# DaehwanKimLab/tophat

Hardware: AMD Instinct MI355X
Metric: paired reads/sec through segment_juncs+long_spanning_reads; junctions.bed diff=0 (higher is better)
Workload: dtype u64

## Files before the change

### tophat_amd/csrc/thj_core.h

```cpp
#pragma once
#include <stdint.h>

#if defined(__HIPCC__)
#define THJ_HD __host__ __device__ __forceinline__
#else
#define THJ_HD inline
#endif

#if defined(THJ_EXP) && defined(__HIPCC__)
static __device__ int thj_exp_flags;
#define THJ_EXPF(b) (thj_exp_flags & (b))
#else
#define THJ_EXPF(b) 0
#endif

namespace thj {

typedef unsigned long long u64;

THJ_HD int popc(u64 x) { return __builtin_popcountll(x); }
THJ_HD int popc32(uint32_t x) { return __builtin_popcount(x); }
THJ_HD int ctz(u64 x) { return __builtin_ctzll(x); }
THJ_HD int clz(u64 x) { return __builtin_clzll(x); }
THJ_HD u64 lowmask(int n) { return n >= 64 ? ~0ull : ((1ull << n) - 1ull); }
// ... 652 lines not shown
    bool run = nseg > 0;
    if (last == 0) run = run && (present & 1u) && !hit_end(h[0]);
    bool check_partner = true;
    if (last != 0 && (present & 1u) && h[0].ref_id == hl.ref_id && hit_anti(h[0]) == hit_anti(hl)) {
        const int dist = hit_anti(h[0]) ? h[0].left - hl.right : hl.left - h[0].right;
        if (dist >= p.min_segment_intron && dist < p.max_segment_intron) check_partner = false;
    }
    res.rescue = run && check_partner && n_mate > 0;
    bool en = run && !res.rescue;
    if (p.bowtie2 && present != 0 && 1 > p.max_seg_multihits) en = false;
#pragma unroll
    for (int s = 0; s + 1 < NS; ++s) {
        const bool has = en && s != last && ((present >> s) & 1u);
        const Hit bh = h[s];
        const bool banti = hit_anti(bh);
        const Hit rh = h[s + 1];
        const bool c1 = ((present >> (s + 1)) & 1u) && banti == hit_anti(rh) && bh.ref_id == rh.ref_id;
        const bool abut = banti ? rh.right == bh.left : bh.right == rh.left;
        const int d1 = banti ? bh.left - rh.right : rh.left - bh.right;
        const bool found = c1 && abut;
        const bool drs = c1 && !abut && d1 >= p.min_segment_intron && d1 < p.max_segment_intron;
        bool rrs = false;
        Hit d = rh;
        if (s + 2 < NS) {
            const Hit rrh = h[s + 2];
            const bool c2 = ((present >> (s + 2)) & 1u) && banti == hit_anti(rrh) && bh.ref_id == rrh.ref_id;
            const int d2 = banti ? bh.left - rrh.right : rrh.left - bh.right;
            rrs = !found && c2 && d2 >= p.min_segment_intron + L && d2 < p.max_segment_intron + L;
            if (rrs) d = rrh;
        }
        const int start = (s + 1) * L - 8;
        int slen = rrs ? L + 16 : 16;
        if (slen > rl - start) slen = rl - start;
        int32_t wl, wr;
        if (!banti) { wl = bh.right - 8; if (wl < 0) wl = 0; wr = d.left + 8; }
        else { wl = d.right - 8; wr = bh.left + 8; }
        const bool ok = has && !found && (drs || rrs) && start >= 0 && slen >= 0;
        emit.task(ok, task_window_word(banti, start, slen), bh.ref_id, (uint32_t)wl, (uint32_t)wr);
        res.n_windows += ok ? 1 : 0;
    }
    return res;
}

enum { SLOT_UNSCANNED = -3 };
template <int MAXM, class Emit>
THJ_HD int flat_rescue(const Params& p, bool has0, const Hit& bh, int size, int rl, const Hit (&mh)[MAXM], int n_mate,
                       const int32_t (&sc)[2 * MAXM], Emit& emit, int& n_windows) {
    const int L = p.segment_length;
    int cl = L - p.segment_mismatches - 3;
    if (cl > 15) cl = 15;
    const bool banti = hit_anti(bh);
    bool alive = has0;
    int pairs = 0, n_pseudo = 0;
    int32_t pl[2 * MAXM];
    bool pv[2 * MAXM];
#pragma unroll
    for (int m = 0; m < MAXM; ++m) {
        const bool compat = alive && m < n_mate && bh.ref_id == mh[m].ref_id && banti != hit_anti(mh[m]);
        const int32_t f = compat ? sc[2 * m] : SLOT_NONE, rv = compat ? sc[2 * m + 1] : SLOT_NONE;
        if (compat && f == SLOT_BREAK) alive = false;
        pairs += (compat && f != SLOT_BREAK && f != SLOT_UNSCANNED) ? 1 : 0;
        pv[2 * m] = compat && alive && f >= 0; pl[2 * m] = f;
        pv[2 * m + 1] = compat && alive && rv >= 0; pl[2 * m + 1] = rv;
        n_pseudo += (pv[2 * m] ? 1 : 0) + (pv[2 * m + 1] ? 1 : 0);
    }
    bool en = has0 && (size == 2 || size == 3);
    if (p.bowtie2 && (1 > p.max_seg_multihits || n_pseudo > p.max_seg_multihits)) en = false;
    const bool far = size == 3;
    const int lo = p.min_segment_intron + (far ? L : 0), hi = p.max_segment_intron + (far ? L : 0);
    bool found = false, inr[2 * MAXM];
    int n = 0;
#pragma unroll
    for (int k = 0; k < 2 * MAXM; ++k) {
        const bool panti = (k & 1) != 0;
        const bool c = pv[k] && banti == panti;
        const int32_t pleft = pl[k], pright = pl[k] + cl;
        const bool abut = banti ? pright == bh.left : bh.right == pleft;
        if (c && abut && !far) found = true;
        const int dist = banti ? bh.left - pright : pleft - bh.right;
        inr[k] = c && dist >= lo && dist < hi;
        n += inr[k] ? 1 : 0;
    }
    const int start = L - 8;
    int slen = far ? L + 16 : 16;
    if (slen > rl - start) slen = rl - start;
    const bool ok_all = en && !found && n > 0 && start >= 0 && slen >= 0;
#pragma unroll
    for (int k = 0; k < 2 * MAXM; ++k) {
        const int32_t pleft = pl[k], pright = pl[k] + cl;
        int32_t wl, wr;
        if (!banti) { wl = bh.right - 8; if (wl < 0) wl = 0; wr = pleft + 8; }
        else { wl = pright - 8; wr = bh.left + 8; }
        const bool ok = ok_all && inr[k];
        emit.task(ok, task_window_word(banti, start, slen), bh.ref_id, (uint32_t)wl, (uint32_t)wr);
        n_windows += ok ? 1 : 0;
    }
    return pairs;
}

template <class Sink>
THJ_HD void gaps_enumerate(const Params& p, const ReadView& v, Sink& sink, int first = 0, int stride = 1) {
    const int L = p.segment_length;
    if (p.bowtie2)
        for (int s = 0; s < v.size; ++s) {
            int n = (!v.rescue || s == 0) ? rv_count_raw(v, s) : rv_count(v, s);
            if (n > p.max_seg_multihits) return;
        }
    for (int s = 0; s < v.size; ++s) {
        rv_foreach_strided(v, s, first, stride, [&](const Hit& bh) {
            bool found = (s == v.size - 1);
            int n_drs = 0, n_rrs = 0;
            const bool banti = hit_anti(bh);
            if (s < v.size - 1) {
                rv_foreach(v, s + 1, [&](const Hit& rh) {
                    if (banti != hit_anti(rh) || bh.ref_id != rh.ref_id) return true;
                    if ((banti && rh.right == bh.left) || (!banti && bh.right == rh.left)) { found = true; return false; }
                    int dist = banti ? bh.left - rh.right : rh.left - bh.right;
                    if (dist >= p.min_segment_intron && dist < p.max_segment_intron) ++n_drs;
                    return true;
                });
            }
            if (!found && s < v.size - 2) {
                rv_foreach(v, s + 2, [&](const Hit& rrh) {
                    if (banti != hit_anti(rrh) || bh.ref_id != rrh.ref_id) return true;
                    int dist = banti ? bh.left - rrh.right : rrh.left - bh.right;
                    if (dist >= p.min_segment_intron + L && dist < p.max_segment_intron + L) ++n_rrs;
                    return true;
                });
            }
            if (!found && (n_drs > 0 || n_rrs > 0)) {
                const bool use_rrs = n_rrs > 0;
                const int lo = p.min_segment_intron + (use_rrs ? L : 0);
                const int hi = p.max_segment_intron + (use_rrs ? L : 0);
                const int start = (s + 1) * L - 8;
                int slen = use_rrs ? L + 16 : 16;
                if (slen > v.rl - start) slen = v.rl - start;
                if (start >= 0 && slen >= 0) {
                    rv_foreach(v, use_rrs ? s + 2 : s + 1, [&](const Hit& d) {
                        if (banti != hit_anti(d) || bh.ref_id != d.ref_id) return true;
                        int dist = banti ? bh.left - d.right : d.left - bh.right;
                        if (dist < lo || dist >= hi) return true;
                        int32_t wl, wr;
                        if (!banti) { wl = bh.right - 8; if (wl < 0) wl = 0; wr = d.left + 8; }
                        else { wl = d.right - 8; wr = bh.left + 8; }
                        sink.window(bh.ref_id, wl, wr, banti, start, slen);
                        return true;
                    });
                }
            }
        });
    }
}

template <class X>
THJ_HD Hit wave_bcast_hit(X& x, const Hit& h, int src) {
    Hit o;
    o.ref_id = x.bcast(h.ref_id, src); o.left = (int32_t)x.bcast((uint32_t)h.left, src);
    o.right = (int32_t)x.bcast((uint32_t)h.right, src); o.meta = x.bcast(h.meta, src);
    return o;
}
THJ_HD Hit wave_lane_hit(const ReadView& v, int s, int lane) {
    Hit h{0, 0, 0, 0};
    if (lane < rv_count_raw(v, s)) h = v.hits[v.so[s] + (uint32_t)lane];
    return h;
}
THJ_HD bool wave_read_fits(const ReadView& v) {
    for (int s = 0; s < v.nseg; ++s) if (rv_count_raw(v, s) > 64) return false;
    return true;
}
template <class X, class Sink>
THJ_HD bool wave_read_enumerate(X& x, const Params& p, ReadView& v, Sink& sink, bool& wants_rescue) {
    const int lane = x.lane;
    const int L = p.segment_length;
    wants_rescue = false;
    v.rescue = false;
    v.check_len = p.segment_length - p.segment_mismatches - 3;
    if (v.check_len > 15) v.check_len = 15;
    if (v.nseg == 0) return false;
    int last = v.nseg - 1;
    while (last > 0 && rv_count_raw(v, last) == 0) --last;
    v.size = last + 1;
    if (last == 0) {
        if (rv_count_raw(v, 0) == 0) return false;
        const Hit h0 = v.hits[v.so[0]];
        if (hit_end(h0)) return false;
    }
    {
        bool found = false;
        if (last != 0) {
            const Hit lh = wave_lane_hit(v, 0, lane);
            const bool have = lane < rv_count_raw(v, 0);
            const Hit D = wave_lane_hit(v, last, lane);
            const int nD = rv_count_raw(v, last);
            for (int j = 0; j < nD; ++j) {
                const Hit rh = wave_bcast_hit(x, D, j);
                if (have && lh.ref_id == rh.ref_id && hit_anti(lh) == hit_anti(rh)) {
                    const int dist = hit_anti(lh) ? lh.left - rh.right : rh.left - lh.right;
                    if (dist >= p.min_segment_intron && dist < p.max_segment_intron) found = true;
                }
            }
        }
        wants_rescue = x.ballot(found) == 0ull && v.n_mate > 0;
    }
    if (wants_rescue) return true;
    if (THJ_EXPF(1 << 27)) return true;
    if (v.nseg >= 2 && !THJ_EXPF(1 << 17))
        for (int i = 0; i + 2 < v.nseg; ++i) {
            const uint32_t lb = v.so[i], le = v.so[i + 1], re = v.so[i + 2];
            if (lb == le || le == re) break;
            const int start = i * L;
            if (start > v.rl) break;
            const int plen = v.rl - start < 2 * L ? v.rl - start : 2 * L;
            const Hit lh = wave_lane_hit(v, i, lane);
            const bool have = (uint32_t)lane < le - lb;
            const Hit C = wave_lane_hit(v, i + 1, lane);
            const int nC = (int)(re - le);
            for (int ri = 0; ri < nC; ++ri) {
                const Hit rh = wave_bcast_hit(x, C, ri);
                if (!have || lh.ref_id != rh.ref_id) continue;
                const bool anti = hit_anti(lh);
                if (anti != hit_anti(rh)) continue;
                const int apparent = anti ? lh.right - rh.left : rh.right - lh.left;
                const int disc = apparent - plen;
                const bool is_del = disc > 0 && disc <= p.max_deletion_length;
                const bool is_ins = disc < 0 && disc >= -p.max_insertion_length;
                if (is_del || is_ins)
                    sink.indel(i, anti ? le + (uint32_t)ri : lb + (uint32_t)lane, anti ? lb + (uint32_t)lane : le + (uint32_t)ri, lane, ri, anti, plen, is_del);
            }
        }
    if (THJ_EXPF(1 << 25)) return true;
    if (p.bowtie2)
        for (int s = 0; s < v.size; ++s) if (rv_count_raw(v, s) > p.max_seg_multihits) return true;
    for (int s = 0; s + 1 < v.size; ++s) {
        const Hit bh = wave_lane_hit(v, s, lane);
        const bool have = lane < rv_count_raw(v, s);
        const bool banti = hit_anti(bh);
        const Hit B = wave_lane_hit(v, s + 1, lane);
        const int nB = rv_count_raw(v, s + 1);
        bool found = false;
        int n_drs = 0, n_rrs = 0;
        for (int c = 0; c < nB; ++c) {
            const Hit rh = wave_bcast_hit(x, B, c);
            if (!have || banti != hit_anti(rh) || bh.ref_id != rh.ref_id) continue;
            if ((banti && rh.right == bh.left) || (!banti && bh.right == rh.left)) found = true;
            const int dist = banti ? bh.left - rh.right : rh.left - bh.right;
            if (dist >= p.min_segment_intron && dist < p.max_segment_intron) ++n_drs;
        }
        Hit C{0, 0, 0, 0};
        int nC = 0;
        if (s < v.size - 2) {
            C = wave_lane_hit(v, s + 2, lane);
            nC = rv_count_raw(v, s + 2);
            if (x.ballot(have && !found) != 0ull)
                for (int c = 0; c < nC; ++c) {
                    const Hit rrh = wave_bcast_hit(x, C, c);
                    if (!have || found || banti != hit_anti(rrh) || bh.ref_id != rrh.ref_id) continue;
                    const int dist = banti ? bh.left - rrh.right : rrh.left - bh.right;
                    if (dist >= p.min_segment_intron + L && dist < p.max_segment_intron + L) ++n_rrs;
                }
        }
        const bool emits = have && !found && (n_drs > 0 || n_rrs > 0);
        const bool use_rrs = n_rrs > 0;
        const int lo = p.min_segment_intron + (use_rrs ? L : 0), hi = p.max_segment_intron + (use_rrs ? L : 0);
        const int start = (s + 1) * L - 8;
        int slen = use_rrs ? L + 16 : 16;
        if (slen > v.rl - start) slen = v.rl - start;
        const bool go = emits && start >= 0 && slen >= 0;
        for (int pass = 0; pass < 2; ++pass) {
            const bool mine = go && (use_rrs ? pass == 1 : pass == 0);
            if (x.ballot(mine) == 0ull) continue;
            const int nT = pass == 0 ? nB : nC;
            for (int c = 0; c < nT; ++c) {
                const Hit d = wave_bcast_hit(x, pass == 0 ? B : C, c);
                if (!mine || banti != hit_anti(d) || bh.ref_id != d.ref_id) continue;
                const int dist = banti ? bh.left - d.right : d.left - bh.right;
                if (dist < lo || dist >= hi) continue;
                int32_t wl, wr;
                if (!banti) { wl = bh.right - 8; if (wl < 0) wl = 0; wr = d.left + 8; }
                else { wl = d.right - 8; wr = bh.left + 8; }
                sink.window(bh.ref_id, wl, wr, banti, start, slen);
            }
        }
    }
    return true;
}

template <class Sink>
THJ_HD void indels_enumerate(const Params& p, const ReadView& v, Sink& sink, int first = 0, int stride = 1) {
    const int L = p.segment_length;
    if (v.nseg < 2) return;
    for (int i = 0; i + 2 < v.nseg; ++i) {
        uint32_t lb = v.so[i], le = v.so[i + 1], re = v.so[i + 2];
        if (lb == le || le == re) return;
        int start = i * L;
        if (start > v.rl) return;
        int plen = v.rl - start < 2 * L ? v.rl - start : 2 * L;
        for (uint32_t li = lb + (uint32_t)first; li < le; li += (uint32_t)stride) {
            Hit lh = v.hits[li];
            for (uint32_t ri = le; ri < re; ++ri) {
                Hit rh = v.hits[ri];
                if (lh.ref_id != rh.ref_id) continue;
                bool anti = hit_anti(lh);
                if (anti != hit_anti(rh)) continue;
                int apparent = anti ? lh.right - rh.left : rh.right - lh.left;
                int disc = apparent - plen;
                bool is_del = disc > 0 && disc <= p.max_deletion_length;
                bool is_ins = disc < 0 && disc >= -p.max_insertion_length;
                if (is_del || is_ins)
                    sink.indel(i, anti ? ri : li, anti ? li : ri, (int)(li - lb), (int)(ri - le), anti, plen, is_del);
            }
        }
    }
}

template <bool WIDE = true, class Sink>
THJ_HD void indel_exec(const Genome& g, const Params& p, const ReadView& v, int i, uint32_t lidx, uint32_t ridx,
                       bool anti, int plen, bool is_del, u64 prio, Sink& sink) {
    const Hit lh = v.hits[lidx], rh = v.hits[ridx];
    if (!WIDE || plen <= 64) {
        if (plen > 64) return;
        PlanesT<u64> rd = Fetch<u64>::read(v.rp, v.W, i * p.segment_length, plen);
        if (anti) rd = Fetch<u64>::rc(rd, plen);
        if (is_del) small_deletion<u64>(g, rd, plen, lh, rh, sink);
        else small_insertion<u64>(g, rd, plen, lh, rh, prio, sink);
    } else if (WIDE) {
        PlanesT<u128> rd = Fetch<u128>::read(v.rp, v.W, i * p.segment_length, plen);
        if (anti) rd = Fetch<u128>::rc(rd, plen);
        if (is_del) small_deletion<u128>(g, rd, plen, lh, rh, sink);
        else small_insertion<u128>(g, rd, plen, lh, rh, prio, sink);
    }
}

template <bool WIDE = true, class Sink>
THJ_HD void window_exec(const Genome& g, const Params& p, const ReadView& v, uint32_t ref_id, int32_t wl, int32_t wr,
                        bool anti, int start, int slen, Sink& sink) {
    if (slen < 2) return;
    if (!WIDE || slen <= 62) {
        if (slen > 62) return;
        PlanesT<u64> sup = Fetch<u64>::read(v.rp, v.W, start, slen);
        if (anti) sup = Fetch<u64>::rc(sup, slen);
        window_scan<u64>(g, p, ref_id, wl, wr, anti, sup, slen, sink);
    } else if (WIDE) {
        PlanesT<u128> sup = Fetch<u128>::read(v.rp, v.W, start, slen);
        if (anti) sup = Fetch<u128>::rc(sup, slen);
        window_scan<u128>(g, p, ref_id, wl, wr, anti, sup, slen, sink);
    }
}

static constexpr int INS_SEQ_BITS = 18;
THJ_HD u64 ins_prio(uint32_t ordinal, int i, int li, int ri) {
    if (li > 63) li = 63;
    if (ri > 63) ri = 63;
    return ((u64)ordinal << 16) | ((u64)(i & 15) << 12) | ((u64)li << 6) | (u64)ri;
}


enum { FUS_FF = 7, FUS_FR = 8, FUS_RF = 9, FUS_RR = 10 };

THJ_HD Planes read_piece(const u64* rp, int W, int rl, bool rc, int off, int len) {
    if (!rc) return r_fetch(rp, W, off, len);
    return rc_piece(r_fetch(rp, W, rl - off - len, len), len);
}
THJ_HD Planes genomic_piece(const Genome& g, uint32_t ref, int64_t start, int rl, bool rc, int off, int len) {
    if (!rc) return g_fetch(g, ref, start + off);
    Planes p = g_fetch(g, ref, start + rl - off - len);
    return rc_piece(p, len);
}

template <int NW>
struct FusEvalT { u64 mL[NW], mR[NW]; int e1, min_err, total_ed; bool lrc, rrc; };
using FusEval = FusEvalT<4>;
template <int NW>
THJ_HD int fusion_eval(const Genome& g, const Params& p, const u64* rp, int W, int rl, bool read_rc, const Hit& lh, const Hit& rh, int dir, FusEvalT<NW>& ev) {
    const int32_t llen = g_len(g, lh.ref_id), rlen = g_len(g, rh.ref_id);
    if (llen == 0 || rlen == 0 || rl > NW * 64) return 0;
    int64_t lstart, rstart;
    const bool lrc = !(dir == FUS_FF || dir == FUS_FR), rrc = !(dir == FUS_FF || dir == FUS_RF);
    ev.lrc = lrc; ev.rrc = rrc;
    if (!lrc) { if (lh.left + rl > llen || lh.left < 0) return 0; lstart = lh.left; }
    else { if (lh.right < rl || lh.right > llen) return 0; lstart = (int64_t)lh.right - rl; }
    if (!rrc) { if (rh.right < rl || rh.right > rlen) return 0; rstart = (int64_t)rh.right - rl; }
    else { if (rh.left + rl > rlen || rh.left < 0) return 0; rstart = rh.left; }
    int tot_r = 0;
#pragma unroll
    for (int w = 0; w < NW; ++w) {
        ev.mL[w] = 0; ev.mR[w] = 0;
        int off = w * 64;
        if (off < rl) {
            int l = rl - off < 64 ? rl - off : 64;
            Planes rd = read_piece(rp, W, rl, read_rc, off, l);
            Planes a = genomic_piece(g, lh.ref_id, lstart, rl, lrc, off, l);
            Planes b = genomic_piece(g, rh.ref_id, rstart, rl, rrc, off, l);
            u64 M = lowmask(l);
            ev.mL[w] = ((a.lo ^ rd.lo) | (a.hi ^ rd.hi) | a.nm | rd.nm) & M;
            ev.mR[w] = ((b.lo ^ rd.lo) | (b.hi ^ rd.hi) | b.nm | rd.nm) & M;
            tot_r += popc(ev.mR[w]);
        }
    }
    ev.e1 = (int)(ev.mL[0] & 1ull) + tot_r - (int)(ev.mR[0] & 1ull);
    ev.total_ed = hit_ed(lh) + hit_ed(rh);
    const int A = p.fusion_anchor_length;
    int mn = rl + 1, cnt = 0, mn_ends = rl + 1, ee = ev.e1;
#pragma unroll
    for (int w = 0; w < NW; ++w) {
        const int q0 = w == 0 ? 1 : w * 64, q1 = rl < (w + 1) * 64 ? rl : (w + 1) * 64;
        u64 l = ev.mL[w] >> (q0 & 63), r = ev.mR[w] >> (q0 & 63);
        for (int q = q0; q < q1; ++q) {
            if (ee < mn) { mn = ee; cnt = 1; } else if (ee == mn) ++cnt;
            if ((q < A || rl - q < A) && ee < mn_ends) mn_ends = ee;
            ee += (int)(l & 1ull) - (int)(r & 1ull);
            l >>= 1; r >>= 1;
        }
    }
    ev.min_err = mn;
    if (mn > ev.total_ed || mn > 2 || mn_ends == mn) return 0;
    return cnt;
}
template <int NW, class F>
THJ_HD void fusion_emit(const FusEvalT<NW>& ev, int rl, const Hit& lh, const Hit& rh, int dir, F f) {
    int ee = ev.e1, k = 0;
#pragma unroll
    for (int w = 0; w < NW; ++w) {
        const int q0 = w == 0 ? 1 : w * 64, q1 = rl < (w + 1) * 64 ? rl : (w + 1) * 64;
        u64 l = ev.mL[w] >> (q0 & 63), r = ev.mR[w] >> (q0 & 63);
        for (int q = q0; q < q1; ++q) {
            if (ee == ev.min_err) {
                uint32_t left = !ev.lrc ? (uint32_t)(lh.left + q - 1) : (uint32_t)(lh.right - q);
                uint32_t right = !ev.rrc ? (uint32_t)(rh.right - (rl - q)) : (uint32_t)(rh.left + (rl - q) - 1);
                uint32_t r1 = lh.ref_id, r2 = rh.ref_id; int tdir = dir;
// ... 118 lines not shown
```

### tophat_amd/csrc/thj_segjuncs.hip

```cpp
#include <hip/hip_runtime.h>
#include <hipcub/hipcub.hpp>

#include <cstdio>
#include <cstdlib>
#include <algorithm>
#include <cstring>
#include <cstddef>
#include <chrono>
#include <vector>

#include "../../include/thj.h"
#include "thj_core.h"
#include "thj_fusion_block.h"
#include "thj_internal.h"

using namespace thj;

static_assert(sizeof(thj_hit) == 16 && sizeof(Hit) == 16, "hit layout");
static_assert(sizeof(thj_params) == sizeof(Params), "params layout");




static constexpr u64 EMPTY = ~0ull;
// ... 379 lines not shown
        sl.scan[(slice + slot) * FLAT_MATES + m] = make_int2(f, rv);
    }
}

__global__ __launch_bounds__(TPB) void thj_k_sj_rescue_flat(Params p, DevBatch b, SjLists sl, int seg_cap, unsigned long long* cnt, unsigned int* n_flat_pairs) {
    __shared__ unsigned int s_ntask, s_stat[2];
    const int tid = threadIdx.x, lane = tid & 63;
    const unsigned int n = sl.frl_cnt[blockIdx.x];
    if (tid == 0) { s_ntask = sl.task_cnt[blockIdx.x]; s_stat[0] = 0; s_stat[1] = 0; }
    __syncthreads();
    const unsigned long long below = lane ? (~0ull >> (64 - lane)) : 0ull;
    const size_t slice = (size_t)blockIdx.x * seg_cap;
    unsigned int my_pairs = 0, my_windows = 0;
    for (unsigned int k0 = 0; k0 < n; k0 += TPB) {
        const unsigned int k = k0 + (unsigned int)tid;
        const bool active = k < n;
        int r = 0, size = 0, n_mate = 0, rlen = 0;
        Hit bh{0, 0, 0, 0}, mh[FLAT_MATES];
        int32_t sc[2 * FLAT_MATES];
#pragma unroll
        for (int m = 0; m < FLAT_MATES; ++m) { mh[m] = Hit{0, 0, 0, 0}; sc[2 * m] = SLOT_NONE; sc[2 * m + 1] = SLOT_NONE; }
        if (active) {
            const uint32_t e = sl.frl[slice + k];
            r = (int)(e & 0x1FFFFFFFu); size = (int)(e >> 29) + 1;
            const uint4 q = ((const uint4*)b.hits)[b.seg_off[(size_t)r * b.nseg]];
            bh.ref_id = q.x; bh.left = (int32_t)q.y; bh.right = (int32_t)q.z; bh.meta = q.w;
            rlen = b.read_len[r];
            const uint32_t m0 = b.mate_off[r];
            n_mate = (int)(b.mate_off[r + 1] - m0);
#pragma unroll
            for (int m = 0; m < FLAT_MATES; ++m)
                if (m < n_mate) {
                    const uint4 w = ((const uint4*)b.mate_hits)[m0 + m];
                    mh[m].ref_id = w.x; mh[m].left = (int32_t)w.y; mh[m].right = (int32_t)w.z; mh[m].meta = w.w;
                    const int2 o = sl.scan[(slice + k) * FLAT_MATES + m];
                    sc[2 * m] = o.x; sc[2 * m + 1] = o.y;
                }
        }
        FlatEmit em{sl.tq + (size_t)blockIdx.x * sl.task_cap, sl.te + (size_t)blockIdx.x * sl.task_cap, &s_ntask, below, (uint32_t)r};
        int nw = 0;
        my_pairs += (unsigned int)flat_rescue<FLAT_MATES>(p, active, bh, size, rlen, mh, n_mate, sc, em, nw);
        my_windows += (unsigned int)nw;
    }
    if (my_pairs) atomicAdd(&s_stat[0], my_pairs);
    if (my_windows) atomicAdd(&s_stat[1], my_windows);
    __syncthreads();
    if (tid == 0) {
        sl.task_cnt[blockIdx.x] = s_ntask;
        if (s_stat[0]) { atomicAdd(&cnt[CNT_RESCUE_PAIRS], (unsigned long long)s_stat[0]); atomicAdd(n_flat_pairs, s_stat[0]); }
        if (s_stat[1]) atomicAdd(&cnt[CNT_WINDOWS], (unsigned long long)s_stat[1]);
    }
}

#ifndef THJ_GEN_HITS
#define THJ_GEN_HITS 8
#endif
static constexpr int GEN_HITS = THJ_GEN_HITS;
static constexpr int MID_HITS = 32;
static constexpr int MID_T = 256;
static constexpr int MID_G = 8;
static constexpr int MID_GRID = 2048;
#ifndef THJ_GEN_G
#define THJ_GEN_G 4
#endif
static constexpr int GEN_G = THJ_GEN_G;
template <int HITS, int T, bool SLICED, int SO, int G = 1>
__global__ __launch_bounds__(T) void thj_k_sj_general(Params p, DevBatch b, RescueList rl, SjLists sl, XTasks x, unsigned long long* cnt) {
    static_assert(G >= 1 && G <= 64 && (G & (G - 1)) == 0 && T % G == 0, "lanes per read");
    constexpr int RPR = T / G;
    constexpr int STRIDE = HITS + 1;
    __shared__ uint32_t q_a[QCAP], q_b[QCAP], q_c[QCAP], q_d[QCAP], q_e[QCAP];
    __shared__ uint4 s_hits[RPR * STRIDE];
    __shared__ uint32_t s_so[RPR * SO];
    __shared__ unsigned int q_n, s_nresc, s_base[3], s_xbase;
    __shared__ unsigned int s_stat[4];
    const int tid = threadIdx.x, lane = tid & 63, slot = tid / G, g = tid % G;
    if (tid < 4) s_stat[tid] = 0;
    if (tid == 0) { q_n = 0; s_nresc = 0; }
    __syncthreads();
    const unsigned long long below = lane ? (~0ull >> (64 - lane)) : 0ull;
    const Queue qq{q_a, q_b, q_c, q_d, q_e, &q_n};
    const unsigned int n = SLICED ? sl.gen_cnt[blockIdx.x] : (*sl.mid_count < (unsigned int)MANY_CAP ? *sl.mid_count : (unsigned int)MANY_CAP);
    const uint32_t* list = SLICED ? sl.gen + (size_t)blockIdx.x * rl.seg_cap : sl.mid_list;
    const unsigned int first = SLICED ? 0u : blockIdx.x * RPR, step = SLICED ? (unsigned int)RPR : gridDim.x * RPR;
    unsigned int my_windows = 0, my_indels = 0;
    for (unsigned int k0 = first; k0 < n; k0 += step) {
        __syncthreads();
        const unsigned int k = k0 + (unsigned int)slot;
        bool active = k < n;
        ReadView v;
        bool do_gaps = false, to_rescue = false;
        int r = 0;
        uint32_t hbase = 0;
        const uint32_t e = active ? list[k] : 0u;
        r = (int)(e & GEN_READ);
        if (SLICED && (e >> 29) != 0u) active = false;
        if (active) {
            v = make_view(b, r);
            const uint32_t h0 = v.so[0], nh = v.so[v.nseg] - h0;
            if (nh <= (uint32_t)HITS) {
                for (int i = g; i <= v.nseg; i += G) s_so[slot * SO + i] = v.so[i] - h0;
                for (uint32_t i = (uint32_t)g; i < nh; i += (uint32_t)G) s_hits[slot * STRIDE + i] = ((const uint4*)b.hits)[h0 + i];
                v.so = s_so + slot * SO; v.hits = (const Hit*)(s_hits + slot * STRIDE); hbase = h0;
            }
        }
        __builtin_amdgcn_fence(__ATOMIC_RELEASE, "wavefront"); __builtin_amdgcn_wave_barrier(); __builtin_amdgcn_fence(__ATOMIC_ACQUIRE, "wavefront");
        if (active) {
            bool wants = false;
            if (G == 1) do_gaps = !THJ_EXPF(1 << 18) && gaps_prepare(p, v, wants);
            else do_gaps = !THJ_EXPF(1 << 18) && gaps_prepare_shared(p, v, wants, g, G, [&](bool f) { return ((__ballot(f) >> (lane - g)) & (~0ull >> (64 - G))) != 0ull; });
            to_rescue = do_gaps && wants;
            if (!to_rescue) {
                QueueSink qs{qq, x, (uint32_t)r, hbase, 0u, 0u};
                if (!THJ_EXPF(1 << 17)) indels_enumerate(p, v, qs, g, G);
                if (do_gaps) gaps_enumerate(p, v, qs, g, G);
                my_windows += qs.n_windows; my_indels += qs.n_indels;
            }
        }
        const bool resc = to_rescue && g == 0;
        if (SLICED) {
            const unsigned int rk = wave_slot(resc, &s_nresc, below);
            if (resc) rl.list[(size_t)blockIdx.x * rl.seg_cap + rk] = (uint32_t)r;
        } else {
            if (tid == 0) s_nresc = 0;
            __syncthreads();
            const unsigned int rk = wave_slot(resc, &s_nresc, below);
            __syncthreads();
            if (tid == 0 && s_nresc) s_base[2] = atomicAdd(&rl.blk_cnt[rl.own_slice], s_nresc);
            __syncthreads();
            if (resc) rl.list[(size_t)rl.own_slice * rl.seg_cap + s_base[2] + rk] = (uint32_t)r;
        }
        flush_tasks(qq, x, &s_xbase, &s_stat[3]);
    }
    if (my_windows) atomicAdd(&s_stat[0], my_windows);
    if (my_indels) atomicAdd(&s_stat[1], my_indels);
    __syncthreads();
    if (tid == 0) {
        if (SLICED) rl.blk_cnt[blockIdx.x] = s_nresc;
        if (s_stat[0]) atomicAdd(&cnt[CNT_WINDOWS], (unsigned long long)s_stat[0]);
        if (s_stat[1]) atomicAdd(&cnt[CNT_INDEL_PAIRS], (unsigned long long)s_stat[1]);
        if (s_stat[3]) atomicAdd(&cnt[CNT_OVF_BLOCKS], (unsigned long long)s_stat[3]);
    }
}

struct SjWave {
    int lane;
    __device__ __forceinline__ unsigned long long ballot(bool p) { return __ballot(p); }
    __device__ __forceinline__ uint32_t bcast(uint32_t v, int src) { return (uint32_t)__builtin_amdgcn_readlane((int)v, __builtin_amdgcn_readfirstlane(src)); }
};
__global__ __launch_bounds__(TPB, 4) void thj_k_segjuncs_shared(Params p, DevBatch b, RescueList rl, XTasks x, unsigned long long* cnt) {
    __shared__ uint32_t q_a[QCAP], q_b[QCAP], q_c[QCAP], q_d[QCAP], q_e[QCAP];
    __shared__ unsigned int q_n;
    __shared__ unsigned int s_stat[4];
    __shared__ Hit s_h[TPB / 64][MANY_HITS_LDS];
    __shared__ uint32_t s_o[TPB / 64][20];
    const int tid = threadIdx.x, lane = tid & 63, wave = tid >> 6;
    if (tid < 4) s_stat[tid] = 0;
    if (tid == 0) q_n = 0;
    __syncthreads();
    const Queue qq{q_a, q_b, q_c, q_d, q_e, &q_n};
    const unsigned int n = *rl.many_count < (unsigned int)MANY_CAP ? *rl.many_count : (unsigned int)MANY_CAP;
    const unsigned int SHARED_BATCH = n / gridDim.x >= 32u ? 32u : n / gridDim.x >= 4u ? n / gridDim.x : 4u;
    __shared__ unsigned int s_next, s_batch, s_nr, s_rbase, s_xbase;
    __shared__ uint32_t s_resc[32];
    if (tid == 0) s_nr = 0;
    unsigned int my_windows = 0, my_indels = 0;
    for (;;) {
        __syncthreads();
        if (tid == 0) { s_next = 0; s_batch = atomicAdd(rl.many_count + 1, 1u); }
        __syncthreads();
        const unsigned int base = s_batch * SHARED_BATCH;
        if (base >= n) break;
        for (;;) {
            unsigned int k = 0;
            if (lane == 0) k = atomicAdd(&s_next, 1u);
            k = (unsigned int)__shfl((int)k, 0);
            if (k >= SHARED_BATCH || base + k >= n) break;
            const int r = (int)rl.many_list[base + k];
            ReadView v = make_view(b, r);
            bool do_gaps = false, wants = false, staged = false;
            uint32_t hbase = 0;
            const uint32_t h0 = v.so[0], nh = v.so[v.nseg] - h0;
            __builtin_amdgcn_fence(__ATOMIC_RELEASE, "wavefront"); __builtin_amdgcn_wave_barrier(); __builtin_amdgcn_fence(__ATOMIC_ACQUIRE, "wavefront");
            if (nh <= (uint32_t)MANY_HITS_LDS && v.nseg < 20) {
                for (uint32_t i = (uint32_t)lane; i < nh; i += 64u) ((uint4*)s_h[wave])[i] = ((const uint4*)b.hits)[h0 + i];
                if (lane <= v.nseg) s_o[wave][lane] = v.so[lane] - h0;
                __builtin_amdgcn_fence(__ATOMIC_RELEASE, "wavefront"); __builtin_amdgcn_wave_barrier(); __builtin_amdgcn_fence(__ATOMIC_ACQUIRE, "wavefront");
                v.hits = s_h[wave]; v.so = s_o[wave]; hbase = h0; staged = true;
            }
            if (THJ_EXPF(1 << 26)) continue;
            if (staged && wave_read_fits(v)) {
                SjWave xw{lane};
                QueueSink qs{qq, x, (uint32_t)r, hbase, 0u, 0u};
                do_gaps = wave_read_enumerate(xw, p, v, qs, wants);
                if (do_gaps && wants) { if (lane == 0) s_resc[atomicAdd(&s_nr, 1u)] = (uint32_t)r; }
                else { my_windows += qs.n_windows; my_indels += qs.n_indels; }
                continue;
            }
            do_gaps = gaps_prepare_shared(p, v, wants, lane, 64, [](bool f) { return __any((int)f) != 0; });
            if (THJ_EXPF(1 << 27)) continue;
            if (do_gaps && wants) {
                if (lane == 0) s_resc[atomicAdd(&s_nr, 1u)] = (uint32_t)r;
            } else {
                QueueSink qs{qq, x, (uint32_t)r, hbase, 0u, 0u};
                if (!THJ_EXPF(1 << 17)) indels_enumerate(p, v, qs, lane, 64);
                if (do_gaps && !THJ_EXPF(1 << 25)) gaps_enumerate(p, v, qs, lane, 64);
                my_windows += qs.n_windows; my_indels += qs.n_indels;
            }
        }
        __syncthreads();
        if (s_nr) {
            if (tid == 0) s_rbase = atomicAdd(&rl.blk_cnt[rl.own_slice], s_nr);
            __syncthreads();
            if ((unsigned int)tid < s_nr) rl.list[(size_t)rl.own_slice * rl.seg_cap + s_rbase + tid] = s_resc[tid];
            __syncthreads();
            if (tid == 0) s_nr = 0;
        }
        flush_tasks(qq, x, &s_xbase, &s_stat[3]);
    }
    if (my_windows) atomicAdd(&s_stat[0], my_windows);
    if (my_indels) atomicAdd(&s_stat[1], my_indels);
    __syncthreads();
    if (tid == 0) {
        if (s_stat[0]) atomicAdd(&cnt[CNT_WINDOWS], (unsigned long long)s_stat[0]);
        if (s_stat[1]) atomicAdd(&cnt[CNT_INDEL_PAIRS], (unsigned long long)s_stat[1]);
        if (s_stat[3]) atomicAdd(&cnt[CNT_OVF_BLOCKS], (unsigned long long)s_stat[3]);
    }
}

static constexpr int RPT = 4;
static constexpr int MSCAN = 128;
static constexpr int RESCUE_GRID = 1024;
static constexpr int HEAVY_CAP = 1 << 18;
static constexpr int MAX_LISTS = 2048;

__global__ __launch_bounds__(TPB, 4) void thj_k_segjuncs_rescue(Genome g, Params p, DevBatch b, RescueList rl, int n_lists, XTasks x, unsigned long long* cnt) {
    __shared__ uint32_t q_a[QCAP], q_b[QCAP], q_c[QCAP], q_d[QCAP], q_e[QCAP];
    __shared__ int32_t s_slots[TPB * RPT * 2];
    __shared__ unsigned int s_off[MAX_LISTS + 1];
    __shared__ unsigned int q_n;
    __shared__ unsigned int s_stat[4];
    __shared__ Genome s_g;
    __shared__ Params s_p;
    typedef hipcub::BlockScan<unsigned int, TPB> Scan;
    __shared__ typename Scan::TempStorage scan_tmp;
    __shared__ unsigned int s_nheavy, s_heavy_base, s_xbase;
    const int tid = threadIdx.x;
    const unsigned long long below = (tid & 63) ? (~0ull >> (64 - (tid & 63))) : 0ull;
    if (tid < 4) s_stat[tid] = 0;
    if (tid == 0) { q_n = 0; s_g = g; s_p = p; }
    unsigned int total;
    {
        constexpr int IPT = MAX_LISTS / TPB;
        unsigned int cnt[IPT], sum = 0, excl;
#pragma unroll
        for (int k = 0; k < IPT; ++k) { const int j = tid * IPT + k; cnt[k] = j < n_lists ? rl.blk_cnt[j] : 0u; sum += cnt[k]; }
        Scan(scan_tmp).ExclusiveSum(sum, excl, total);
#pragma unroll
        for (int k = 0; k < IPT; ++k) { s_off[tid * IPT + k] = excl; excl += cnt[k]; }
        if (tid == 0) s_off[MAX_LISTS] = total;
    }
    __syncthreads();
    const Queue qq{q_a, q_b, q_c, q_d, q_e, &q_n};
    const unsigned int per_round = gridDim.x * TPB;
    const unsigned int rounds = (total + per_round - 1) / per_round;
    unsigned int my_pairs = 0, my_windows = 0, my_indels = 0;
    for (unsigned int it = 0; it < rounds; ++it) {
        const unsigned int i = (it * gridDim.x + blockIdx.x) * TPB + tid;
        const bool active = i < total;
        __syncthreads();
        ReadView v;
        bool do_gaps = false, heavy = false;
        int r = 0;
        if (active) {
            int lo = 0, hi = n_lists;
            while (hi - lo > 1) { const int mid = (lo + hi) >> 1; if (s_off[mid] <= i) lo = mid; else hi = mid; }
            r = (int)rl.list[(size_t)lo * rl.seg_cap + (i - s_off[lo])];
            v = make_view(b, r);
            heavy = (int64_t)rv_count_raw(v, 0) * v.n_mate > RPT && v.n_mate <= MSCAN && !THJ_EXPF(1 << 24);
        }
        unsigned int hk = 0;
        {
            if (tid == 0) s_nheavy = 0;
            __syncthreads();
            hk = wave_slot(heavy, &s_nheavy, below);
            __syncthreads();
            if (tid == 0 && s_nheavy) s_heavy_base = atomicAdd(rl.heavy_count, s_nheavy);
            __syncthreads();
            hk += s_heavy_base;
            heavy = heavy && hk < (unsigned int)HEAVY_CAP;
        }
        if (active) {
            QueueSink qs{qq, x, (uint32_t)r, 0u, 0u, 0u};
            if (heavy) rl.heavy_list[hk] = (uint32_t)r;
            if (!heavy) indels_enumerate(p, v, qs);
            const bool wants = true;
            gaps_prepare_listed(p, v);
            do_gaps = true;
            if (do_gaps && !heavy) {
                if (wants) {
                    const int n_left = rv_count_raw(v, 0);
                    const bool fits = (int64_t)n_left * v.n_mate <= RPT;
                    int32_t* mine = s_slots + tid * RPT * 2;
                    unsigned int local = 0;
                    int32_t c0_f = SLOT_NONE, c0_rv = SLOT_NONE, c1_f = SLOT_NONE, c1_rv = SLOT_NONE; bool c0_ok = false, c1_ok = false; unsigned int sc_have = 0;
                    for (int l = 0; l < n_left; ++l)
                        for (int m = 0; m < v.n_mate; ++m) {
                            int32_t f = SLOT_NONE, rv = SLOT_NONE;
                            if (THJ_EXPF(1 << 22)) { }
                            else {
                                const Hit lh = v.hits[v.so[0] + l], rh = v.mate[m];
                                if (lh.ref_id == rh.ref_id && hit_anti(lh) != hit_anti(rh)) {
                                    bool scanned;
                                    if (m == 0) {
                                        if (!(sc_have & 1u)) { c0_ok = rescue_scan(g, p, v.rp, v.W, v.rl, rh, c0_f, c0_rv); sc_have |= 1u; }
                                        f = c0_f; rv = c0_rv; scanned = c0_ok;
                                    } else if (m == 1) {
                                        if (!(sc_have & 2u)) { c1_ok = rescue_scan(g, p, v.rp, v.W, v.rl, rh, c1_f, c1_rv); sc_have |= 2u; }
                                        f = c1_f; rv = c1_rv; scanned = c1_ok;
                                    } else scanned = rescue_scan(g, p, v.rp, v.W, v.rl, rh, f, rv);
                                    if (scanned) ++local;
                                }
                            }
                            if (fits) { mine[2 * (l * v.n_mate + m)] = f; mine[2 * (l * v.n_mate + m) + 1] = rv; }
                            if (f == SLOT_BREAK) break;
                        }
                    my_pairs += local;
                    v.rescue = true;
                    v.slots = fits ? mine : nullptr;
                    v.lazy_g = &s_g; v.lazy_p = &s_p;
                }
                if (!THJ_EXPF(1 << 23)) gaps_enumerate(p, v, qs);
            }
            my_windows += qs.n_windows; my_indels += qs.n_indels;
        }
        flush_tasks(qq, x, &s_xbase, &s_stat[3]);
    }
    if (my_pairs) atomicAdd(&s_stat[2], my_pairs);
    if (my_windows) atomicAdd(&s_stat[0], my_windows);
    if (my_indels) atomicAdd(&s_stat[1], my_indels);
    __syncthreads();
    if (tid == 0) {
        if (s_stat[0]) atomicAdd(&cnt[CNT_WINDOWS], (unsigned long long)s_stat[0]);
        if (s_stat[1]) atomicAdd(&cnt[CNT_INDEL_PAIRS], (unsigned long long)s_stat[1]);
// ... 1204 lines not shown
```

Baseline: 2.085 billion.

## Flatten wave pair loops over all hit pairs instead of per-lane broadcast loops

Rewrites the wave-level read enumeration so each lane evaluates one (left, right) hit pair per trip, flattening the k×kB product into 64-wide chunks. A float-derived magic multiply, checked by a static_assert, splits the flat index into pair indices. Per-left results are gathered through ballots and lane masks instead of serial readlane broadcasts of whole hits. This targets the serial per-right-hit broadcast loop that left lanes idle when segment hit counts are small. In exchange, every pair now does LDS loads, and there are extra ballots per trip. It also uses readfirstlane for the wave index and the work counter so they stay scalar.

```diff
diff --git a/tophat_amd/csrc/thj_core.h b/tophat_amd/csrc/thj_core.h
--- a/tophat_amd/csrc/thj_core.h
+++ b/tophat_amd/csrc/thj_core.h
@@ -828,25 +828,42 @@
     }
 }
 
-template <class X>
-THJ_HD Hit wave_bcast_hit(X& x, const Hit& h, int src) {
-    Hit o;
-    o.ref_id = x.bcast(h.ref_id, src); o.left = (int32_t)x.bcast((uint32_t)h.left, src);
-    o.right = (int32_t)x.bcast((uint32_t)h.right, src); o.meta = x.bcast(h.meta, src);
-    return o;
-}
-THJ_HD Hit wave_lane_hit(const ReadView& v, int s, int lane) {
-    Hit h{0, 0, 0, 0};
-    if (lane < rv_count_raw(v, s)) h = v.hits[v.so[s] + (uint32_t)lane];
-    return h;
-}
 THJ_HD bool wave_read_fits(const ReadView& v) {
     for (int s = 0; s < v.nseg; ++s) if (rv_count_raw(v, s) > 64) return false;
     return true;
 }
+THJ_HD Hit pair_hit(const Hit* q) {
+#if defined(__HIP_DEVICE_COMPILE__)
+    return *(const Hit*)__builtin_assume_aligned(q, 16);
+#else
+    return *q;
+#endif
+}
+THJ_HD uint32_t pair_magic(int kp) { return (uint32_t)(1048576.0f / (float)kp) + 1u; }
+constexpr bool pair_magic_exact(uint32_t dm) {
+    for (uint32_t kp = 1; kp <= 64u; ++kp) {
+        const unsigned long long M = (1u << 20) / kp + 1u + dm;
+        for (uint32_t a = 1; a <= 64u; ++a)
+            if ((((unsigned long long)(a * kp - 1u) * M) >> 20) != a - 1u || (((unsigned long long)(a * kp) * M) >> 20) != a) return false;
+    }
+    return true;
+}
+static_assert(pair_magic_exact(0u) && pair_magic_exact(1u), "pair_magic: (t M) >> 20 is not t / k'");
+THJ_HD uint32_t pair_mul(uint32_t a, uint32_t b) { return (a & 0xFFFFFFu) * (b & 0xFFFFFFu); }
+struct PairLeft { uint32_t T0, T1; u64 m0, m1; };
+THJ_HD PairLeft pair_left(uint32_t lane, int kp) {
+    const uint32_t base = pair_mul(lane, (uint32_t)kp);
+    const unsigned sh = base & 63u;
+    const u64 km = lowmask(kp);
+    return PairLeft{base >> 6, (base >> 6) + 1u, km << sh, sh ? km >> (64u - sh) : 0ull};
+}
+THJ_HD bool pair_left_any(const PairLeft& q, u64 w, uint32_t trip) {
+    const u64 m = trip == q.T0 ? q.m0 : trip == q.T1 ? q.m1 : 0ull;
+    return (w & m) != 0ull;
+}
 template <class X, class Sink>
 THJ_HD bool wave_read_enumerate(X& x, const Params& p, ReadView& v, Sink& sink, bool& wants_rescue) {
-    const int lane = x.lane;
+    const uint32_t lane = (uint32_t)x.lane;
     const int L = p.segment_length;
     wants_rescue = false;
     v.rescue = false;
@@ -864,19 +881,20 @@
     {
         bool found = false;
         if (last != 0) {
-            const Hit lh = wave_lane_hit(v, 0, lane);
-            const bool have = lane < rv_count_raw(v, 0);
-            const Hit D = wave_lane_hit(v, last, lane);
-            const int nD = rv_count_raw(v, last);
-            for (int j = 0; j < nD; ++j) {
-                const Hit rh = wave_bcast_hit(x, D, j);
-                if (have && lh.ref_id == rh.ref_id && hit_anti(lh) == hit_anti(rh)) {
-                    const int dist = hit_anti(lh) ? lh.left - rh.right : rh.left - lh.right;
-                    if (dist >= p.min_segment_intron && dist < p.max_segment_intron) found = true;
-                }
-            }
-        }
-        wants_rescue = x.ballot(found) == 0ull && v.n_mate > 0;
+            const Hit* A = v.hits + v.so[0];
+            const Hit* D = v.hits + v.so[last];
+            const int kp = rv_count_raw(v, last);
+            const uint32_t n = (uint32_t)rv_count_raw(v, 0) * (uint32_t)kp, M = pair_magic(kp);
+            for (uint32_t t0 = 0; t0 < n && !found; t0 += 64u) {
+                const uint32_t t = t0 + lane, tt = t < n ? t : 0u;
+                const uint32_t a = pair_mul(tt, M) >> 20, b = tt - pair_mul(a, (uint32_t)kp);
+                const Hit lh = pair_hit(A + a), rh = pair_hit(D + b);
+                const int dist = (hit_anti(lh) ? lh.left : rh.left) - (hit_anti(lh) ? rh.right : lh.right);
+                const bool ok = (t < n) & (lh.ref_id == rh.ref_id) & (hit_anti(lh) == hit_anti(rh)) & (dist >= p.min_segment_intron) & (dist < p.max_segment_intron);
+                found = x.ballot(ok) != 0ull;
+            }
+        }
+        wants_rescue = !found && v.n_mate > 0;
     }
     if (wants_rescue) return true;
     if (THJ_EXPF(1 << 27)) return true;
@@ -887,70 +905,86 @@
             const int start = i * L;
             if (start > v.rl) break;
             const int plen = v.rl - start < 2 * L ? v.rl - start : 2 * L;
-            const Hit lh = wave_lane_hit(v, i, lane);
-            const bool have = (uint32_t)lane < le - lb;
-            const Hit C = wave_lane_hit(v, i + 1, lane);
-            const int nC = (int)(re - le);
-            for (int ri = 0; ri < nC; ++ri) {
-                const Hit rh = wave_bcast_hit(x, C, ri);
-                if (!have || lh.ref_id != rh.ref_id) continue;
+            const uint32_t kp = re - le, n = (le - lb) * kp, M = pair_magic((int)kp);
+            for (uint32_t t0 = 0; t0 < n; t0 += 64u) {
+                const uint32_t t = t0 + lane, tt = t < n ? t : 0u;
+                const uint32_t li = pair_mul(tt, M) >> 20, ri = tt - pair_mul(li, kp);
+                const Hit lh = pair_hit(v.hits + lb + li), rh = pair_hit(v.hits + le + ri);
                 const bool anti = hit_anti(lh);
-                if (anti != hit_anti(rh)) continue;
-                const int apparent = anti ? lh.right - rh.left : rh.right - lh.left;
+                const int apparent = (anti ? lh.right : rh.right) - (anti ? rh.left : lh.left);
                 const int disc = apparent - plen;
-                const bool is_del = disc > 0 && disc <= p.max_deletion_length;
-                const bool is_ins = disc < 0 && disc >= -p.max_insertion_length;
-                if (is_del || is_ins)
-                    sink.indel(i, anti ? le + (uint32_t)ri : lb + (uint32_t)lane, anti ? lb + (uint32_t)lane : le + (uint32_t)ri, lane, ri, anti, plen, is_del);
+                const bool is_del = (disc > 0) & (disc <= p.max_deletion_length);
+                const bool is_ins = (disc < 0) & (disc >= -p.max_insertion_length);
+                if ((t < n) & (lh.ref_id == rh.ref_id) & (anti == hit_anti(rh)) & (is_del | is_ins))
+                    sink.indel(i, anti ? le + ri : lb + li, anti ? lb + li : le + ri, (int)li, (int)ri, anti, plen, is_del);
             }
         }
     if (THJ_EXPF(1 << 25)) return true;
     if (p.bowtie2)
         for (int s = 0; s < v.size; ++s) if (rv_count_raw(v, s) > p.max_seg_multihits) return true;
     for (int s = 0; s + 1 < v.size; ++s) {
-        const Hit bh = wave_lane_hit(v, s, lane);
-        const bool have = lane < rv_count_raw(v, s);
-        const bool banti = hit_anti(bh);
-        const Hit B = wave_lane_hit(v, s + 1, lane);
-        const int nB = rv_count_raw(v, s + 1);
-        bool found = false;
-        int n_drs = 0, n_rrs = 0;
-        for (int c = 0; c < nB; ++c) {
-            const Hit rh = wave_bcast_hit(x, B, c);
-            if (!have || banti != hit_anti(rh) || bh.ref_id != rh.ref_id) continue;
-            if ((banti && rh.right == bh.left) || (!banti && bh.right == rh.left)) found = true;
-            const int dist = banti ? bh.left - rh.right : rh.left - bh.right;
-            if (dist >= p.min_segment_intron && dist < p.max_segment_intron) ++n_drs;
-        }
-        Hit C{0, 0, 0, 0};
-        int nC = 0;
-        if (s < v.size - 2) {
-            C = wave_lane_hit(v, s + 2, lane);
-            nC = rv_count_raw(v, s + 2);
-            if (x.ballot(have && !found) != 0ull)
-                for (int c = 0; c < nC; ++c) {
-                    const Hit rrh = wave_bcast_hit(x, C, c);
-                    if (!have || found || banti != hit_anti(rrh) || bh.ref_id != rrh.ref_id) continue;
-                    const int dist = banti ? bh.left - rrh.right : rrh.left - bh.right;
-                    if (dist >= p.min_segment_intron + L && dist < p.max_segment_intron + L) ++n_rrs;
-                }
-        }
-        const bool emits = have && !found && (n_drs > 0 || n_rrs > 0);
-        const bool use_rrs = n_rrs > 0;
-        const int lo = p.min_segment_intron + (use_rrs ? L : 0), hi = p.max_segment_intron + (use_rrs ? L : 0);
+        const int k = rv_count_raw(v, s);
+        if (k == 0) continue;
+        const Hit* A = v.hits + v.so[s];
+        const int kB = rv_count_raw(v, s + 1), kC = s + 2 < v.size ? rv_count_raw(v, s + 2) : 0;
+        u64 found = 0ull, drs = 0ull, rrs = 0ull;
+        if (kB > 0) {
+            const Hit* B = v.hits + v.so[s + 1];
+            const uint32_t n = (uint32_t)k * (uint32_t)kB, M = pair_magic(kB);
+            const PairLeft mine = pair_left(lane, kB);
+            bool my_found = false, my_drs = false;
+            for (uint32_t t0 = 0, trip = 0; t0 < n; t0 += 64u, ++trip) {
+                const uint32_t t = t0 + lane, tt = t < n ? t : 0u;
+                const uint32_t a = pair_mul(tt, M) >> 20, b = tt - pair_mul(a, (uint32_t)kB);
+                const Hit bh = pair_hit(A + a), rh = pair_hit(B + b);
+                const bool banti = hit_anti(bh);
+                const bool c = (t < n) & (banti == hit_anti(rh)) & (bh.ref_id == rh.ref_id);
+                const int dist = (banti ? bh.left : rh.left) - (banti ? rh.right : bh.right);
+                const u64 w_abut = x.ballot(c & (dist == 0));
+                const u64 w_near = x.ballot(c & (dist >= p.min_segment_intron) & (dist < p.max_segment_intron));
+                if (w_abut != 0ull) my_found |= pair_left_any(mine, w_abut, trip);
+                if (w_near != 0ull) my_drs |= pair_left_any(mine, w_near, trip);
+            }
+            found = x.ballot(my_found);
+            drs = x.ballot(my_drs);
+        }
+        const u64 unfound = lowmask(k) & ~found;
+        if (kC > 0 && unfound != 0ull) {
+            const Hit* C = v.hits + v.so[s + 2];
+            const uint32_t n = (uint32_t)k * (uint32_t)kC, M = pair_magic(kC);
+            const PairLeft mine = pair_left(lane, kC);
+            bool my_rrs = false;
+            for (uint32_t t0 = 0, trip = 0; t0 < n; t0 += 64u, ++trip) {
+                const uint32_t t = t0 + lane, tt = t < n ? t : 0u;
+                const uint32_t a = pair_mul(tt, M) >> 20, b = tt - pair_mul(a, (uint32_t)kC);
+                const Hit bh = pair_hit(A + a), rrh = pair_hit(C + b);
+                const bool banti = hit_anti(bh);
+                const int dist = (banti ? bh.left : rrh.left) - (banti ? rrh.right : bh.right);
+                const u64 w_far = x.ballot((t < n) & (banti == hit_anti(rrh)) & (bh.ref_id == rrh.ref_id) &
+                                           (dist >= p.min_segment_intron + L) & (dist < p.max_segment_intron + L));
+                if (w_far != 0ull) my_rrs |= pair_left_any(mine, w_far, trip);
+            }
+            rrs = x.ballot(my_rrs);
+        }
+        rrs &= unfound;
         const int start = (s + 1) * L - 8;
-        int slen = use_rrs ? L + 16 : 16;
-        if (slen > v.rl - start) slen = v.rl - start;
-        const bool go = emits && start >= 0 && slen >= 0;
+        if (start < 0) continue;
         for (int pass = 0; pass < 2; ++pass) {
-            const bool mine = go && (use_rrs ? pass == 1 : pass == 0);
-            if (x.ballot(mine) == 0ull) continue;
-            const int nT = pass == 0 ? nB : nC;
-            for (int c = 0; c < nT; ++c) {
-                const Hit d = wave_bcast_hit(x, pass == 0 ? B : C, c);
-                if (!mine || banti != hit_anti(d) || bh.ref_id != d.ref_id) continue;
-                const int dist = banti ? bh.left - d.right : d.left - bh.right;
-                if (dist < lo || dist >= hi) continue;
+            const u64 go = pass == 0 ? unfound & drs & ~rrs : rrs;
+            int slen = pass == 0 ? 16 : L + 16;
+            if (slen > v.rl - start) slen = v.rl - start;
+            if (go == 0ull || slen < 0) continue;
+            const int kT = pass == 0 ? kB : kC;
+            const Hit* T = v.hits + v.so[s + 1 + pass];
+            const int lo = p.min_segment_intron + (pass == 0 ? 0 : L), hi = p.max_segment_intron + (pass == 0 ? 0 : L);
+            const uint32_t n = (uint32_t)k * (uint32_t)kT, M = pair_magic(kT);
+            for (uint32_t t0 = 0; t0 < n; t0 += 64u) {
+                const uint32_t t = t0 + lane, tt = t < n ? t : 0u;
+                const uint32_t a = pair_mul(tt, M) >> 20, b = tt - pair_mul(a, (uint32_t)kT);
+                const Hit bh = pair_hit(A + a), d = pair_hit(T + b);
+                const bool banti = hit_anti(bh);
+                const int dist = (banti ? bh.left : d.left) - (banti ? d.right : bh.right);
+                if (!((t < n) & (((go >> a) & 1ull) != 0ull) & (banti == hit_anti(d)) & (bh.ref_id == d.ref_id) & (dist >= lo) & (dist < hi))) continue;
                 int32_t wl, wr;
                 if (!banti) { wl = bh.right - 8; if (wl < 0) wl = 0; wr = d.left + 8; }
                 else { wl = d.right - 8; wr = bh.left + 8; }
diff --git a/tophat_amd/csrc/thj_segjuncs.hip b/tophat_amd/csrc/thj_segjuncs.hip
--- a/tophat_amd/csrc/thj_segjuncs.hip
+++ b/tophat_amd/csrc/thj_segjuncs.hip
@@ -555,9 +555,9 @@
     __shared__ uint32_t q_a[QCAP], q_b[QCAP], q_c[QCAP], q_d[QCAP], q_e[QCAP];
     __shared__ unsigned int q_n;
     __shared__ unsigned int s_stat[4];
-    __shared__ Hit s_h[TPB / 64][MANY_HITS_LDS];
+    __shared__ alignas(16) Hit s_h[TPB / 64][MANY_HITS_LDS];
     __shared__ uint32_t s_o[TPB / 64][20];
-    const int tid = threadIdx.x, lane = tid & 63, wave = tid >> 6;
+    const int tid = threadIdx.x, lane = tid & 63, wave = __builtin_amdgcn_readfirstlane(tid >> 6);
     if (tid < 4) s_stat[tid] = 0;
     if (tid == 0) q_n = 0;
     __syncthreads();
@@ -577,7 +577,7 @@
         for (;;) {
             unsigned int k = 0;
             if (lane == 0) k = atomicAdd(&s_next, 1u);
-            k = (unsigned int)__shfl((int)k, 0);
+            k = (unsigned int)__builtin_amdgcn_readfirstlane((int)k);
             if (k >= SHARED_BATCH || base + k >= n) break;
             const int r = (int)rl.many_list[base + k];
             ReadView v = make_view(b, r);
@@ -593,6 +593,7 @@
             }
             if (THJ_EXPF(1 << 26)) continue;
             if (staged && wave_read_fits(v)) {
+                v.hits = s_h[wave]; v.so = s_o[wave];
                 SjWave xw{lane};
                 QueueSink qs{qq, x, (uint32_t)r, hbase, 0u, 0u};
                 do_gaps = wave_read_enumerate(xw, p, v, qs, wants);
```

Result: faster. 2.156 billion, median of 6 (+3.4%).
